# arrufat/zignal

Measured on NVIDIA H100. Metric: Mpixels/sec Gaussian-blur 8K RGBA f32, higher is better.
Workload: dtype f32

## Files before the change

zignal_b200/csrc/zb_conv_fused.cu:

```cuda
#include "zb_conv.h"
#include "zb_device.cuh"
#include "zb_shard.h"
#include "zb_tma.cuh"

namespace zb {

namespace {

constexpr int TW = 256;
constexpr int CHUNK = 8;
constexpr int G = TW / 8 + 2;
constexpr int STAGE_BYTES = G * CHUNK * 128;
constexpr int RING_ROWS = 24;
constexpr int RING_ROW_BYTES = TW * 16;
constexpr int RING_BYTES = RING_ROWS * RING_ROW_BYTES;
constexpr int NTHREADS = 256;
constexpr int MAX_HALF = 8;
constexpr int MAXK = 2 * MAX_HALF + 1;
constexpr int STAGES = 2;
constexpr int SMEM_BYTES = STAGES * STAGE_BYTES + RING_BYTES + 64 + 1024;

struct FusedParams {
    float kx[MAXK];
    float ky[MAXK];
    const float4* src;
    float4* dst;
    unsigned long long src_pitch_px, dst_pitch_px;
    int rows, cols, border;
    int ngroups;
    int n_strips;
    int n_units;
    int strip_lo, strip_hi;
    int n_segs, seg_chunks, seg_extra;
    int e_segs, e_chunks, e_extra;
    int row0, row1;
    int fix_rows;
    int fix_left;
    int fix_right;
    int tma_row_off;
    int edge_fast;
    int lsrc[8];
    int rsrc[8];
};

struct ShardParams {
    const float4* up_rows;
    const float4* down_rows;
    unsigned long long up_pitch_px, down_pitch_px;
    int half;
    ShardLink link;
};

template <bool ROTATE>
__device__ __forceinline__ void unit_at(const FusedParams& p, int u, int& strip, int& ra, int& rb) {
    const int n_inner = p.strip_hi - p.strip_lo;
    int seg, chunks, extra;
    if (u < p.n_segs * n_inner) {
        seg = u / n_inner;
        strip = p.strip_lo + (u - seg * n_inner);
        if constexpr (ROTATE) seg = seg + 1 == p.n_segs ? 0 : seg + 1;
        chunks = p.seg_chunks;
        extra = p.seg_extra;
    } else {
        const int n_edge = p.n_strips - n_inner;
        u -= p.n_segs * n_inner;
        seg = u / n_edge;
        const int e = u - seg * n_edge;
        strip = e < p.strip_lo ? e : e - p.strip_lo + p.strip_hi;
        chunks = p.e_chunks;
        extra = p.e_extra;
    }
    ra = p.row0 + (seg * chunks + min(seg, extra)) * CHUNK;
    rb = min(ra + (chunks + (seg < extra ? 1 : 0)) * CHUNK, p.row1);
}

template <bool EXACT>
__device__ __forceinline__ void mac4(float4& acc, const float4& v, float k) {
    if constexpr (EXACT) {
        acc.x = __fadd_rn(acc.x, __fmul_rn(v.x, k));
        acc.y = __fadd_rn(acc.y, __fmul_rn(v.y, k));
        acc.z = __fadd_rn(acc.z, __fmul_rn(v.z, k));
        acc.w = __fadd_rn(acc.w, __fmul_rn(v.w, k));
    } else {
        acc.x = fmaf(v.x, k, acc.x);
        acc.y = fmaf(v.y, k, acc.y);
        acc.z = fmaf(v.z, k, acc.z);
        acc.w = fmaf(v.w, k, acc.w);
    }
}

template <bool SHARD>
__device__ __noinline__ void fixup_stage(uint32_t stage, int y0, int xs0, bool fix_x, bool fix_rows, const FusedParams& p,
                                         int nb_lo, int nb_hi) {
    const int xlimit = p.ngroups * 8;
    auto stage_addr = [&](int rr, int xx) {
        const uint32_t line = (uint32_t)(rr * G + (xx >> 3));
        return stage + line * 128 + ((((uint32_t)xx & 7u) ^ (line & 7u)) << 4);
    };
    if (fix_x && p.edge_fast) {
        fix_x = false;
        if (threadIdx.x < 128) {
            const int side = threadIdx.x >> 6, rr = (threadIdx.x >> 3) & 7, e = threadIdx.x & 7;
            const int y = y0 + rr;
            bool row_ok = y >= 0 && y < p.rows;
            if constexpr (SHARD) row_ok = row_ok || (y < 0 && y >= nb_lo) || (y >= p.rows && y < nb_hi);
            const bool edge = side == 0 ? xs0 < 0 : xs0 + G * 8 > p.cols;
            if (row_ok && edge) {
                const int s_dst = side == 0 ? e : p.cols - xs0 + e;
                const int s_src = side == 0 ? p.lsrc[e] : p.rsrc[e] - xs0;
                if (s_dst < G * 8) sts128(stage_addr(rr, s_dst), lds128(stage_addr(rr, s_src)));
            }
        }
    }
    if (fix_x) {
        const int nleft = xs0 < 0 ? min(-xs0, G * 8) : 0;
        const int r0 = max(0, xlimit - xs0);
        const int r1 = min(G * 8, p.cols - xs0 + MAX_HALF);
        const int per_row = nleft + max(0, r1 - r0);
        for (int idx = threadIdx.x; idx < CHUNK * per_row; idx += NTHREADS) {
            const int rr = idx / per_row, e = idx - rr * per_row;
            const int xx = e < nleft ? e : r0 + (e - nleft);
            const int y = y0 + rr, x = xs0 + xx;
            const float4* rowp = p.src + (long long)y * (long long)p.src_pitch_px;
            if (y < 0 || y >= p.rows) {
                if constexpr (SHARD) {
                    if (y < nb_lo || y >= nb_hi) continue;
                } else {
                    continue;
                }
            }
            const int rx = resolve_index(x, p.cols, p.border);
            float4 v = make_float4(0.f, 0.f, 0.f, 0.f);
            if (rx >= 0) {
                const int sx = rx - xs0;
                if (rx < xlimit && sx >= 0 && sx < G * 8) v = lds128(stage_addr(rr, sx));
                else v = __ldg(rowp + rx);
            }
            sts128(stage_addr(rr, xx), v);
        }
    }
    if (fix_rows) {
        for (int idx = threadIdx.x; idx < CHUNK * G * 8; idx += NTHREADS) {
            const int rr = idx / (G * 8);
            const int xx = idx - rr * (G * 8);
            const int y = y0 + rr, x = xs0 + xx;
            if (y >= 0 && y < p.rows) continue;
            if constexpr (SHARD) {
                if (y >= nb_lo && y < nb_hi) continue;
            }
            const int ry = resolve_index(y, p.rows, p.border);
            const int rx = resolve_index(x, p.cols, p.border);
            float4 v = make_float4(0.f, 0.f, 0.f, 0.f);
            if (ry >= 0 && rx >= 0) v = __ldg(p.src + (size_t)ry * p.src_pitch_px + rx);
            sts128(stage_addr(rr, xx), v);
        }
    }
}

template <int HALF, bool EXACT, int SLOT>
__device__ __forceinline__ void v_pass(uint32_t v_col, const FusedParams& p, float4* out, bool col_ok, int rows_left) {
    constexpr int K = 2 * HALF + 1;
    constexpr int NLOAD = CHUNK + 2 * HALF;
    float4 acc[8];
#pragma unroll
    for (int o = 0; o < 8; ++o) acc[o] = make_float4(0.f, 0.f, 0.f, 0.f);
#pragma unroll
    for (int j = 0; j < NLOAD; ++j) {
        const int sr = (SLOT * CHUNK + 8 - HALF + j) % RING_ROWS;
        const float4 v = lds128(v_col + (uint32_t)(sr * RING_ROW_BYTES));
#pragma unroll
        for (int o = 0; o < 8; ++o) {
            const int ti = j - o;
            if (ti >= 0 && ti < K) mac4<EXACT>(acc[o], v, p.ky[ti]);
        }
    }
    if (col_ok) {
#pragma unroll
        for (int o = 0; o < 8; ++o)
            if (o < rows_left) __stcs(out + (size_t)o * p.dst_pitch_px, acc[o]);
    }
}

template <int HALF, bool EXACT, bool SHARD>
__device__ __forceinline__ uint32_t fused_units(const CUtensorMap& tmap, const FusedParams& p, unsigned nbr, int k_begin, int k_end, uint32_t count0) {
    constexpr int K = 2 * HALF + 1;
    constexpr int NLOAD = CHUNK + 2 * HALF;
    extern __shared__ unsigned char smem_raw[];
    const uint32_t smem0 = (smem_u32(smem_raw) + 1023u) & ~1023u;
    const uint32_t ring = smem0 + STAGES * STAGE_BYTES;
    const uint32_t bar0 = ring + RING_BYTES;

    const int tid = threadIdx.x;
    const long long u_first = (long long)blockIdx.x + (long long)k_begin * gridDim.x;
    const long long u_last = (long long)blockIdx.x + (long long)k_end * gridDim.x;
    const int n_units = (int)min((long long)p.n_units, u_last);
    if (u_first >= n_units) return count0;
    auto touches_neighbour = [&](int y) { return ((nbr & 1u) && y < 0) || ((nbr & 2u) && y + CHUNK > p.rows); };

    int pu = (int)u_first, pi = 0;
    uint32_t pcount = count0;
    auto produce = [&]() {
        if (pu >= n_units) return;
        int strip, ra, rb;
        unit_at<SHARD>(p, pu, strip, ra, rb);
        const int n_in = (rb - ra + CHUNK - 1) / CHUNK + 2;
        const uint32_t st = pcount % STAGES;
        const int y = ra - CHUNK + CHUNK * pi;
        fence_proxy_async();
        mbar_arrive_expect_tx(bar0 + 8 * st, STAGE_BYTES);
        tma_load_3d(smem0 + st * STAGE_BYTES, &tmap, 0, strip * (TW / 8) - 1, y + p.tma_row_off, bar0 + 8 * st);
        ++pcount;
        if (++pi == n_in) { pi = 0; pu += gridDim.x; }
    };
    if (tid == 0)
        for (int i = 0; i < STAGES; ++i) produce();

    const int ht = tid & 31, hr = tid >> 5;
    const int vx = tid;
    const uint32_t v_col = ring + (uint32_t)(vx >> 3) * 128u + ((((uint32_t)vx & 7u) ^ (((uint32_t)vx >> 3) & 7u)) << 4);
    const uint32_t h_ring_col = ring + (uint32_t)ht * 128u;
    const uint32_t h_key = (uint32_t)ht & 7u;

    uint32_t ccount = count0;

    for (int unit = (int)u_first; unit < n_units; unit += gridDim.x) {
        int strip, ra, rb;
        unit_at<SHARD>(p, unit, strip, ra, rb);
        const int x0 = strip * TW;
        const int n_out = (rb - ra + CHUNK - 1) / CHUNK;
        const int n_in = n_out + 2;
        const int g0 = x0 / 8 - 1;

        for (int i = 0; i < n_in; ++i, ++ccount) {
            const uint32_t st = ccount % STAGES;
            const uint32_t stage = smem0 + st * STAGE_BYTES;
            while (!mbar_try_wait(bar0 + 8 * st, (ccount / STAGES) & 1u)) {}
            const int y0 = ra - CHUNK + CHUNK * i;
            bool fix_r = p.fix_rows && (y0 < 0 || y0 + CHUNK > p.rows);
            if constexpr (SHARD) {
                if (touches_neighbour(y0)) fix_r = false;
            }
            const bool fix_x = (p.fix_left && g0 < 0) || (p.fix_right && (g0 + G) * 8 > p.ngroups * 8);
            if (fix_r || fix_x) {
                fixup_stage<SHARD>(stage, y0, g0 * 8, fix_x, fix_r, p, (nbr & 1u) ? INT_MIN : 0, (nbr & 2u) ? INT_MAX : p.rows);
                __syncthreads();
            }

            {
                const uint32_t line0 = (uint32_t)(hr * G + ht);
                uint32_t lbase[3];
#pragma unroll
                for (int l = 0; l < 3; ++l) lbase[l] = stage + (line0 + l) * 128u + (((line0 + l) & 7u) << 4);
                const uint32_t rrow = h_ring_col + (uint32_t)(((i % 3) * CHUNK + hr) * RING_ROW_BYTES);
                float4 acc[8];
#pragma unroll
                for (int o = 0; o < 8; ++o) acc[o] = make_float4(0.f, 0.f, 0.f, 0.f);
#pragma unroll
                for (int j = 0; j < NLOAD; ++j) {
                    const int pidx = 8 - HALF + j;
                    const float4 v = lds128(lbase[pidx >> 3] ^ (((uint32_t)pidx & 7u) << 4));
#pragma unroll
                    for (int o = 0; o < 8; ++o) {
                        const int ti = j - o;
                        if (ti >= 0 && ti < K) mac4<EXACT>(acc[o], v, p.kx[ti]);
                    }
                }
#pragma unroll
                for (int o = 0; o < 8; ++o) sts128(rrow + ((((uint32_t)o) ^ h_key) << 4), acc[o]);
            }
            __syncthreads();

            if (tid == 0) produce();

            if (i >= 2) {
                const int c = i - 2;
                const int x = x0 + vx;
                const int yb = ra + CHUNK * c;
                float4* out = p.dst + (size_t)yb * p.dst_pitch_px + x;
                const bool col_ok = x < p.cols;
                switch (c % 3) {
                    case 0: v_pass<HALF, EXACT, 0>(v_col, p, out, col_ok, rb - yb); break;
                    case 1: v_pass<HALF, EXACT, 1>(v_col, p, out, col_ok, rb - yb); break;
                    default: v_pass<HALF, EXACT, 2>(v_col, p, out, col_ok, rb - yb); break;
                }
            }
            __syncthreads();
        }
    }
    return ccount;
}

template <int HALF, bool EXACT, bool SHARD>
__device__ __forceinline__ void fused_sep_rgbaf32_body(const CUtensorMap& tmap, const FusedParams& p, const ShardParams* sp) {
    extern __shared__ unsigned char smem_raw[];
    const uint32_t smem0 = (smem_u32(smem_raw) + 1023u) & ~1023u;
    const uint32_t bar0 = smem0 + STAGES * STAGE_BYTES + RING_BYTES;
    const int tid = threadIdx.x;
    if (tid == 0) {
        asm volatile("prefetch.tensormap [%0];" ::"l"(&tmap) : "memory");
        for (int i = 0; i < STAGES; ++i) mbar_init(bar0 + 8 * i, 1);
        fence_barrier_init();
    }
    if constexpr (!SHARD) {
        __syncthreads();
        fused_units<HALF, EXACT, false>(tmap, p, 0u, 0, INT_MAX / 2048, 0u);
    } else {
        ShardCtrl* me = sp->link.self;
        const unsigned long long epoch = sp->link.epoch;
        const unsigned nbr = (sp->up_rows ? 1u : 0u) | (sp->down_rows ? 2u : 0u);
        const int per_side = sp->half * p.cols;
        const int total = (sp->up_rows ? per_side : 0) + (sp->down_rows ? per_side : 0);
        constexpr int BATCH = 12;
        const int rem = p.n_units % (int)gridDim.x;
        const int n_copiers = (int)gridDim.x - rem;
        const int ci = (int)blockIdx.x - rem;
        const bool copier = ci >= 0 && (long long)ci * NTHREADS * BATCH < total;
        if (tid == 0) {
            if (blockIdx.x == 0) {
                me->dbg[0] = global_timer_ns();
                if (sp->link.up) st_release_sys(&sp->link.up->ready_from[1], epoch);
                if (sp->link.down) st_release_sys(&sp->link.down->ready_from[0], epoch);
            }
            if (copier) {
                if (sp->up_rows) shard_wait_ge(&me->ready_from[0], epoch, me);
                if (sp->down_rows) shard_wait_ge(&me->ready_from[1], epoch, me);
                if (ci == 0) me->dbg[1] = global_timer_ns();
            }
        }
        __syncthreads();
        if (copier) {
            for (int base = ci * NTHREADS * BATCH; base < total; base += n_copiers * NTHREADS * BATCH) {
                float4 v[BATCH];
                float4* dstp[BATCH];
    #pragma unroll
                for (int k = 0; k < BATCH; ++k) {
                    int e = base + k * NTHREADS + tid;
                    dstp[k] = nullptr;
                    if (e < total) {
                        const bool upper = sp->up_rows && e < per_side;
                        if (!upper && sp->up_rows) e -= per_side;
                        const int r = e / p.cols, x = e - r * p.cols;
                        if (upper) {
                            v[k] = *(sp->up_rows + (size_t)r * sp->up_pitch_px + x);
                            dstp[k] = const_cast<float4*>(p.src) + (long long)(r - sp->half) * (long long)p.src_pitch_px + x;
                        } else {
                            v[k] = *(sp->down_rows + (size_t)r * sp->down_pitch_px + x);
                            dstp[k] = const_cast<float4*>(p.src) + (long long)(p.rows + r) * (long long)p.src_pitch_px + x;
                        }
                    }
                }
    #pragma unroll
                for (int k = 0; k < BATCH; ++k)
                    if (dstp[k]) *dstp[k] = v[k];
            }
            asm volatile("fence.proxy.async;" ::: "memory");
            __syncthreads();
        }
        if (tid == 0) {
            __threadfence();
            if (atomicAdd(&me->halo_reads[0], 1u) == gridDim.x - 1u) {
                me->halo_reads[0] = 0;
                me->dbg[2] = global_timer_ns();
                __threadfence();
                st_release_sys(&me->halo_landed, epoch);
                if (sp->up_rows) st_release_sys(&sp->link.up->done_from[1], epoch);
                if (sp->down_rows) st_release_sys(&sp->link.down->done_from[0], epoch);
            }
        }
        const long long first_halo_unit = (long long)max(0, p.n_segs - 2) * p.n_strips;
        const int k_split = first_halo_unit <= (long long)blockIdx.x ? 0 : (int)((first_halo_unit - blockIdx.x + gridDim.x - 1) / gridDim.x);
        const uint32_t count = fused_units<HALF, EXACT, true>(tmap, p, nbr, 0, k_split, 0u);
        if ((long long)blockIdx.x + (long long)k_split * gridDim.x < (long long)p.n_units) {
            if (tid == 0) {
                shard_wait_ge(&me->halo_landed, epoch, me);
                asm volatile("fence.proxy.async;" ::: "memory");
            }
            __syncthreads();
            fused_units<HALF, EXACT, true>(tmap, p, nbr, k_split, INT_MAX / 2048, count);
        }
        if (tid == 0) {
            ShardCtrl* me = sp->link.self;
            __threadfence();
            if (atomicAdd(&me->exit_ticket, 1u) == gridDim.x - 1u) {
                me->exit_ticket = 0;
                me->dbg[3] = global_timer_ns();
                if (sp->link.up) shard_wait_ge(&me->done_from[0], sp->link.epoch, me);
                if (sp->link.down) shard_wait_ge(&me->done_from[1], sp->link.epoch, me);
                me->dbg[4] = global_timer_ns();
            }
        }
    }
}


template <int HALF, bool EXACT>
__global__ void __launch_bounds__(NTHREADS, 1)
fused_sep_rgbaf32_kernel(const __grid_constant__ CUtensorMap tmap, const __grid_constant__ FusedParams p) {
    fused_sep_rgbaf32_body<HALF, EXACT, false>(tmap, p, nullptr);
}

template <int HALF, bool EXACT>
__global__ void __launch_bounds__(NTHREADS, 1)
fused_sep_rgbaf32_shard_kernel(const __grid_constant__ CUtensorMap tmap, const __grid_constant__ FusedParams p,
                               const __grid_constant__ ShardParams sp) {
    fused_sep_rgbaf32_body<HALF, EXACT, true>(tmap, p, &sp);
}

template <int HALF>
int launch_fused(const CUtensorMap& tmap, const FusedParams& p, const ShardParams* sp, int grid, bool exact, cudaStream_t s) {
    if (sp) {
        auto k = exact ? fused_sep_rgbaf32_shard_kernel<HALF, true> : fused_sep_rgbaf32_shard_kernel<HALF, false>;
        ZB_CUDA(cudaFuncSetAttribute(k, cudaFuncAttributeMaxDynamicSharedMemorySize, SMEM_BYTES));
        k<<<grid, NTHREADS, SMEM_BYTES, s>>>(tmap, p, *sp);
    } else {
        auto k = exact ? fused_sep_rgbaf32_kernel<HALF, true> : fused_sep_rgbaf32_kernel<HALF, false>;
        ZB_CUDA(cudaFuncSetAttribute(k, cudaFuncAttributeMaxDynamicSharedMemorySize, SMEM_BYTES));
        k<<<grid, NTHREADS, SMEM_BYTES, s>>>(tmap, p);
    }
    ZB_LAUNCHED();
    return ZB_OK;
}

int launch_half(int half, const CUtensorMap& tmap, const FusedParams& p, const ShardParams* sp, int grid, bool exact, cudaStream_t s) {
    switch (half) {
        case 1: return launch_fused<1>(tmap, p, sp, grid, exact, s);
        case 2: return launch_fused<2>(tmap, p, sp, grid, exact, s);
        case 3: return launch_fused<3>(tmap, p, sp, grid, exact, s);
        case 4: return launch_fused<4>(tmap, p, sp, grid, exact, s);
        case 5: return launch_fused<5>(tmap, p, sp, grid, exact, s);
        case 6: return launch_fused<6>(tmap, p, sp, grid, exact, s);
        case 7: return launch_fused<7>(tmap, p, sp, grid, exact, s);
        case 8: return launch_fused<8>(tmap, p, sp, grid, exact, s);
    }
    return ZB_ERR_UNSUPPORTED;
}

}

static int encode_block_map(EncodeTiledFn encode, CUtensorMap& tmap, void* data, int ngroups, int rows, uint64_t stride_px) {
    const cuuint64_t gdim[3] = {32, (cuuint64_t)ngroups, (cuuint64_t)rows};
    const cuuint64_t gstr[2] = {128, (cuuint64_t)stride_px * 16};
    const cuuint32_t box[3] = {32, (cuuint32_t)G, (cuuint32_t)CHUNK};
    const cuuint32_t estr[3] = {1, 1, 1};
    CUresult cr = encode(&tmap, CU_TENSOR_MAP_DATA_TYPE_FLOAT32, 3, data, gdim, gstr, box, estr, CU_TENSOR_MAP_INTERLEAVE_NONE,
                         CU_TENSOR_MAP_SWIZZLE_128B, CU_TENSOR_MAP_L2_PROMOTION_L2_256B, CU_TENSOR_MAP_FLOAT_OOB_FILL_NONE);
    if (cr != CUDA_SUCCESS) {
        snprintf(t_last_error, sizeof(t_last_error), "cuTensorMapEncodeTiled failed: %d", (int)cr);
        return ZB_ERR_UNSUPPORTED;
    }
    return ZB_OK;
}

constexpr long long EDGE_COST_NUM = 5, EDGE_COST_DEN = 4;

static void plan_units(int nrows, int sm_count, FusedParams& p) {
    const long long chunks = (nrows + CHUNK - 1) / CHUNK;
    const long long max_segs = chunks / 8 < 1 ? 1 : (chunks / 8 < sm_count ? chunks / 8 : sm_count);
    const long long n_inner = p.strip_hi - p.strip_lo, n_edge = p.n_strips - n_inner;
    auto steps = [&](long long segs) { return (chunks + segs - 1) / segs + 2; };
    long long best_cost = -1, best_units = 0, best_s = 1, best_e = 1;
    for (long long s = 1; s <= max_segs; ++s) {
        const long long waves = (s * p.n_strips + sm_count - 1) / sm_count;
        long long e = s;
        if (n_edge > 0) {
            long long e_max = (waves * sm_count - s * n_inner) / n_edge;
            if (e_max > max_segs) e_max = max_segs;
            while (e < e_max && EDGE_COST_NUM * steps(e) > EDGE_COST_DEN * steps(s)) ++e;
        }
        const long long inner = n_inner > 0 ? EDGE_COST_DEN * steps(s) : 0, edge = n_edge > 0 ? EDGE_COST_NUM * steps(e) : 0;
        const long long cost = waves * (inner > edge ? inner : edge), units = s * n_inner + e * n_edge;
        if (best_cost < 0 || cost < best_cost || (cost == best_cost && units < best_units)) {
            best_cost = cost;
            best_units = units;
            best_s = s;
            best_e = e;
        }
    }
    p.n_units = (int)best_units;
    p.n_segs = (int)best_s;
    p.seg_chunks = (int)(chunks / best_s);
    p.seg_extra = (int)(chunks % best_s);
    p.e_segs = (int)best_e;
    p.e_chunks = (int)(chunks / best_e);
    p.e_extra = (int)(chunks % best_e);
}

static int fused_prepare(const zb_image* src, zb_image* dst, const float* kx, int nx, const float* ky, int ny, int border, int row0, int row1,
                         bool bands, FusedParams& p, CUtensorMap& tmap, int& grid, int& half_out, EncodeTiledFn& encode) {
    const int half_x = nx / 2, half_y = ny / 2;
    const int half = half_x > half_y ? half_x : half_y;
    if (half < 1 || half > MAX_HALF) return ZB_ERR_UNSUPPORTED;
    if (src->cols < 16 || src->rows < 16) return ZB_ERR_UNSUPPORTED;
    if (images_overlap(src, dst, 16)) return ZB_ERR_UNSUPPORTED;
    if (((uintptr_t)src->data & 15u) || ((uintptr_t)dst->data & 15u)) return ZB_ERR_UNSUPPORTED;
    for (int i = 0; i < nx; ++i) if (fabsf(kx[i]) < 1e-10f) return ZB_ERR_UNSUPPORTED;
    for (int i = 0; i < ny; ++i) if (fabsf(ky[i]) < 1e-10f) return ZB_ERR_UNSUPPORTED;
    encode = encode_tiled_fn();
    if (!encode) return ZB_ERR_UNSUPPORTED;
    DeviceInfo di;
    int rc = device_info(&di);
    if (rc) return rc;
    if (di.smem_optin < (size_t)SMEM_BYTES) return ZB_ERR_UNSUPPORTED;

    memset(&p, 0, sizeof(p));
    for (int i = 0; i < nx; ++i) p.kx[i + (half - half_x)] = kx[i];
    for (int i = 0; i < ny; ++i) p.ky[i + (half - half_y)] = ky[i];
    p.src = (const float4*)src->data;
    p.dst = (float4*)dst->data;
    p.src_pitch_px = src->stride;
    p.dst_pitch_px = dst->stride;
    p.rows = (int)src->rows;
    p.cols = (int)src->cols;
    p.border = border;
    p.ngroups = p.cols / 8;
    p.n_strips = (p.cols + TW - 1) / TW;
    p.row0 = row0 < 0 ? 0 : row0;
    p.row1 = (row1 < 0 || row1 > p.rows) ? p.rows : row1;
    if (p.row1 <= p.row0) { grid = 0; return ZB_OK; }
    const int nrows = p.row1 - p.row0;
    p.fix_rows = border != ZB_BORDER_ZERO;
    p.fix_left = border != ZB_BORDER_ZERO;
    p.fix_right = (border != ZB_BORDER_ZERO) || (p.cols % 8 != 0);
    p.strip_lo = 0;
    p.strip_hi = p.n_strips;
    if (bands) {
        const BandPlan plan = plan_bands(nrows, p.n_strips, di.sm_count, g_tune_band_rows.load());
        p.n_segs = plan.n_bands;
        p.seg_chunks = plan.band_rows / CHUNK;
        p.n_units = p.n_segs * p.n_strips;
    } else {
        if (p.fix_left) p.strip_lo = 1;
        while (p.fix_right && p.strip_hi > p.strip_lo && (p.strip_hi - 1) * (TW / 8) - 1 + G > p.ngroups) --p.strip_hi;
        if (p.strip_hi <= p.strip_lo) { p.strip_lo = 0; p.strip_hi = p.n_strips; }
        plan_units(nrows, di.sm_count, p);
    }
    p.edge_fast = g_tune_edge_fast.load() && (border == ZB_BORDER_REPLICATE || border == ZB_BORDER_MIRROR) && p.cols % 8 == 0 && p.cols >= 16;
    for (int e = 0; e < 8; ++e) {
        const int xl = e - 8, xr = p.cols + e;
        p.lsrc[e] = 8 + (border == ZB_BORDER_REPLICATE ? 0 : -xl);
        p.rsrc[e] = border == ZB_BORDER_REPLICATE ? p.cols - 1 : 2 * (p.cols - 1) - xr;
    }

    if ((rc = encode_block_map(encode, tmap, src->data, p.ngroups, p.rows, src->stride))) return rc;
    grid = p.n_units < di.sm_count ? p.n_units : di.sm_count;
    half_out = half;
    return ZB_OK;
}

int conv_separable_fused_rgbaf32(const zb_image* src, zb_image* dst, const float* kx, int nx, const float* ky, int ny, int border,
                                 bool exact, cudaStream_t s, int row0, int row1) {
    FusedParams p;
    CUtensorMap tmap;
    EncodeTiledFn encode;
    int grid = 0, half = 0;
    int rc = fused_prepare(src, dst, kx, nx, ky, ny, border, row0, row1, false, p, tmap, grid, half, encode);
    if (rc || grid == 0) return rc;
    t_last_kernel = exact ? "fused_sep_rgbaf32_exact" : "fused_sep_rgbaf32";
    return launch_half(half, tmap, p, nullptr, grid, exact, s);
}

int conv_separable_fused_rgbaf32_shard(const zb_image* src, zb_image* dst, const float* kx, int nx, const float* ky, int ny, int border,
                                       bool exact, const PeerBlock& up, const PeerBlock& down, uint32_t halo_cap, const ShardLink& link,
                                       cudaStream_t s) {
    if (src->rows % CHUNK != 0 || halo_cap < (uint32_t)CHUNK) return ZB_ERR_UNSUPPORTED;
    FusedParams p;
    CUtensorMap tmap;
    EncodeTiledFn encode;
    int grid = 0, half = 0;
    int rc = fused_prepare(src, dst, kx, nx, ky, ny, border, 0, -1, true, p, tmap, grid, half, encode);
    if (rc) return rc;
    if (grid == 0) return ZB_ERR_UNSUPPORTED;
    const uint32_t hv = (uint32_t)(ny / 2);
    if ((up.data && (up.rows < hv || ((uintptr_t)up.data & 15u))) || (down.data && (down.rows < hv || ((uintptr_t)down.data & 15u))))
        return ZB_ERR_UNSUPPORTED;
    void* ext = (char*)src->data - (size_t)halo_cap * src->stride * 16;
    if ((rc = encode_block_map(encode, tmap, ext, p.ngroups, (int)(src->rows + 2 * halo_cap), src->stride))) return rc;
    p.tma_row_off = (int)halo_cap;
    p.fix_rows = 1;
    ShardParams sp;
    memset(&sp, 0, sizeof(sp));
    sp.half = (int)hv;
    if (up.data && hv) {
        sp.up_rows = (const float4*)up.data + (size_t)(up.rows - hv) * up.stride;
        sp.up_pitch_px = up.stride;
    }
    if (down.data && hv) {
        sp.down_rows = (const float4*)down.data;
        sp.down_pitch_px = down.stride;
    }
    sp.link = link;
    if (!sp.up_rows) sp.link.up = nullptr;
    if (!sp.down_rows) sp.link.down = nullptr;
    {
        DeviceInfo di;
        if ((rc = device_info(&di))) return rc;
        grid = di.sm_count;
    }
    t_last_kernel = exact ? "fused_sep_rgbaf32_shard_exact" : "fused_sep_rgbaf32_shard";
    return launch_half(half, tmap, p, &sp, grid, exact, s);
}

}
```

zignal_b200/csrc/zb_internal.h:

```cpp
#pragma once
#include <cuda.h>
#include <cuda_runtime.h>

#include <atomic>
#include <cstdint>
#include <cstdio>
#include <cstring>

#include "../../include/zignal_b200.h"

namespace zb {

extern std::atomic<uint64_t> g_launches;
extern thread_local char t_last_error[512];
extern thread_local const char* t_last_kernel;
extern std::atomic<int> g_exact_f32;
extern std::atomic<int> g_force_generic;
extern std::atomic<int> g_tune_band_rows;
extern std::atomic<int> g_tune_host_band_rows;
extern std::atomic<int> g_tune_edge_fast;
extern std::atomic<int> g_tune_sobel_tile;
extern std::atomic<int> g_tune_jacobi_cluster;
extern std::atomic<int> g_tune_u8_dp;
extern std::atomic<int> g_tune_u8_fmath;
extern std::atomic<int> g_tune_hough_threads;
extern std::atomic<int> g_tune_hough_max_cols;
extern std::atomic<int> g_tune_dither_publish;

int set_cuda_error(cudaError_t e, const char* what, const char* file, int line);

#define ZB_CUDA(expr)                                                                    \
    do {                                                                                 \
        cudaError_t _e = (expr);                                                         \
        if (_e != cudaSuccess) return ::zb::set_cuda_error(_e, #expr, __FILE__, __LINE__); \
    } while (0)

#define ZB_LAUNCHED()                                                                      \
    do {                                                                                   \
        ::zb::g_launches.fetch_add(1, std::memory_order_relaxed);                          \
        cudaError_t _e = cudaGetLastError();                                               \
        if (_e != cudaSuccess) return ::zb::set_cuda_error(_e, "kernel launch", __FILE__, __LINE__); \
    } while (0)

struct DeviceInfo {
    int ordinal = -1;
    int sm_count = 0;
    size_t smem_optin = 0;
};
int device_info(DeviceInfo* out);
typedef CUresult (*EncodeTiledFn)(CUtensorMap*, CUtensorMapDataType, cuuint32_t, void*, const cuuint64_t*, const cuuint64_t*,
                                  const cuuint32_t*, const cuuint32_t*, CUtensorMapInterleave, CUtensorMapSwizzle,
                                  CUtensorMapL2promotion, CUtensorMapFloatOOBfill);
EncodeTiledFn encode_tiled_fn();

static inline int channels_of(int pixfmt) {
    switch (pixfmt) {
        case ZB_PIX_U8: case ZB_PIX_F32: return 1;
        case ZB_PIX_RGB8: return 3;
        case ZB_PIX_RGBA8: case ZB_PIX_RGBAF32: return 4;
    }
    return 0;
}
static inline size_t channel_bytes(int pixfmt) { return (pixfmt == ZB_PIX_F32 || pixfmt == ZB_PIX_RGBAF32) ? 4 : 1; }
static inline size_t pixel_bytes(int pixfmt) { return (size_t)channels_of(pixfmt) * channel_bytes(pixfmt); }
static inline bool is_float_fmt(int pixfmt) { return pixfmt == ZB_PIX_F32 || pixfmt == ZB_PIX_RGBAF32; }

struct Scratch {
    void* p = nullptr;
    cudaStream_t s = nullptr;
    ~Scratch() { if (p) cudaFreeAsync(p, s); }
    int alloc(size_t bytes, cudaStream_t stream);
    template <typename T> T* as() const { return (T*)p; }
// ... 34 lines not shown
```

zignal_b200/csrc/zb_runtime.cu:

```cuda
#include <mutex>

#include "zb_internal.h"

namespace zb {

std::atomic<uint64_t> g_launches{0};
thread_local char t_last_error[512] = "";
thread_local const char* t_last_kernel = "";
std::atomic<int> g_exact_f32{0};
std::atomic<int> g_force_generic{0};
std::atomic<int> g_tune_band_rows{256};
std::atomic<int> g_tune_host_band_rows{256};
std::atomic<int> g_tune_u8_fmath{1};
std::atomic<int> g_tune_u8_dp{1};
std::atomic<int> g_tune_rotate_tile{1};
std::atomic<int> g_tune_edge_fast{1};
std::atomic<int> g_tune_sobel_tile{1};
std::atomic<int> g_tune_jacobi_cluster{1};

int set_cuda_error(cudaError_t e, const char* what, const char* file, int line) {
    snprintf(t_last_error, sizeof(t_last_error), "%s: %s (%s:%d)", cudaGetErrorName(e), what, file, line);
    if (e == cudaErrorMemoryAllocation) return ZB_ERR_OUT_OF_MEMORY;
    return ZB_ERR_DEVICE_FAILURE;
}

static std::mutex g_mu;
static DeviceInfo g_dev[64];
static EncodeTiledFn g_encode = nullptr;

int device_info(DeviceInfo* out) {
    int dev = 0;
    ZB_CUDA(cudaGetDevice(&dev));
    if (dev < 0 || dev >= 64) return ZB_ERR_DEVICE_FAILURE;
    std::lock_guard<std::mutex> lk(g_mu);
    if (g_dev[dev].ordinal != dev) {
        cudaDeviceProp prop;
        ZB_CUDA(cudaGetDeviceProperties(&prop, dev));
        g_dev[dev].sm_count = prop.multiProcessorCount;
        g_dev[dev].smem_optin = prop.sharedMemPerBlockOptin;
        cudaMemPool_t pool;
        ZB_CUDA(cudaDeviceGetDefaultMemPool(&pool, dev));
        uint64_t thresh = UINT64_MAX;
        ZB_CUDA(cudaMemPoolSetAttribute(pool, cudaMemPoolAttrReleaseThreshold, &thresh));
        g_dev[dev].ordinal = dev;
    }
    *out = g_dev[dev];
    return ZB_OK;
}

EncodeTiledFn encode_tiled_fn() {
    std::lock_guard<std::mutex> lk(g_mu);
    if (!g_encode) {
        void* fn = nullptr;
        cudaDriverEntryPointQueryResult qres;
        if (cudaGetDriverEntryPoint("cuTensorMapEncodeTiled", &fn, cudaEnableDefault, &qres) == cudaSuccess &&
            qres == cudaDriverEntryPointSuccess)
            g_encode = (EncodeTiledFn)fn;
    }
    return g_encode;
}

int Scratch::alloc(size_t bytes, cudaStream_t stream) {
    s = stream;
    if (bytes == 0) bytes = 16;
    ZB_CUDA(cudaMallocAsync(&p, bytes, stream));
    return ZB_OK;
}

}

using namespace zb;

extern "C" {

int zb_version(void) { return ZB_VERSION_MAJOR * 1000 + ZB_VERSION_MINOR; }

const char* zb_status_name(int status) {
    switch (status) {
        case ZB_OK: return "Ok";
        case ZB_ERR_DIMENSION_MISMATCH: return "DimensionMismatch";
        case ZB_ERR_INVALID_SIGMA: return "InvalidSigma";
        case ZB_ERR_UNSUPPORTED: return "Unsupported";
        case ZB_ERR_NOT_CONVERGED: return "NotConverged";
        case ZB_ERR_INVALID_ARGUMENT: return "InvalidArgument";
        case ZB_ERR_OUT_OF_MEMORY: return "OutOfMemory";
        case ZB_ERR_DEVICE_FAILURE: return "DeviceFailure";
        case ZB_ERR_INVALID_SCALE_FACTOR: return "InvalidScaleFactor";
        case ZB_ERR_INVALID_DIMENSIONS: return "InvalidDimensions";
        case ZB_ERR_NO_TARGET_SET: return "NoTargetSet";
        case ZB_ERR_NO_SOURCE_SET: return "NoSourceSet";
        case ZB_ERR_INSUFFICIENT_DATA: return "InsufficientData";
        case ZB_ERR_INVALID_COMPONENTS: return "InvalidComponents";
        case ZB_ERR_INVALID_THRESHOLD: return "InvalidThreshold";
        case ZB_ERR_INVALID_PERCENTILE: return "InvalidPercentile";
        case ZB_ERR_INVALID_TRIM: return "InvalidTrim";
        case ZB_ERR_IMAGE_TOO_SMALL: return "ImageTooSmall";
        case ZB_ERR_NOT_SQUARE: return "NotSquare";
        case ZB_ERR_NOT_SYMMETRIC: return "NotSymmetric";
        case ZB_ERR_NOT_FINITE: return "NotFinite";
        case ZB_ERR_INVALID_CUTOFF: return "InvalidCutoff";
        case ZB_ERR_INVALID_RADIUS: return "InvalidRadius";
        case ZB_ERR_INVALID_KERNEL_SIZE: return "InvalidKernelSize";
        case ZB_ERR_INVALID_B_PARAMETER: return "InvalidBParameter";
        case ZB_ERR_WINDOW_SIZE_MUST_BE_ODD: return "WindowSizeMustBeOdd";
        case ZB_ERR_WINDOW_SIZE_TOO_SMALL: return "WindowSizeTooSmall";
        case ZB_ERR_OUT_OF_BOUNDS: return "OutOfBounds";
        case ZB_ERR_NO_PALETTE_COLORS: return "NoPaletteColors";
    }
    return "Unknown";
}

const char* zb_last_error(void) { return t_last_error; }
const char* zb_last_kernel(void) { return t_last_kernel; }
uint64_t zb_kernel_launch_count(void) { return g_launches.load(); }
int zb_set_exact_f32(int on) { g_exact_f32.store(on ? 1 : 0); return ZB_OK; }
int zb_set_force_generic(int on) { g_force_generic.store(on ? 1 : 0); return ZB_OK; }
int zb_tune(const char* key, int value) {
    if (!key) return ZB_ERR_INVALID_ARGUMENT;
    if (!strcmp(key, "conv.u8_fmath")) { g_tune_u8_fmath.store(value ? 1 : 0); return ZB_OK; }
    if (!strcmp(key, "conv.u8_dp")) { g_tune_u8_dp.store(value ? 1 : 0); return ZB_OK; }
    if (!strcmp(key, "conv.edge_fast")) { g_tune_edge_fast.store(value ? 1 : 0); return ZB_OK; }
    if (!strcmp(key, "sobel.tile")) { g_tune_sobel_tile.store(value ? 1 : 0); return ZB_OK; }
    if (!strcmp(key, "jacobi.cluster")) { g_tune_jacobi_cluster.store(value ? 1 : 0); return ZB_OK; }
    if (!strcmp(key, "rotate.tile")) { g_tune_rotate_tile.store(value ? 1 : 0); return ZB_OK; }
    if (!strcmp(key, "host.band_rows")) { if (value < 0) return ZB_ERR_INVALID_ARGUMENT; g_tune_host_band_rows.store(value); return ZB_OK; }
    if (!strcmp(key, "conv.band_rows")) { if (value < 64) return ZB_ERR_INVALID_ARGUMENT; g_tune_band_rows.store(value); return ZB_OK; }
    if (!strcmp(key, "hough.threads")) {
        if (value < 128 || value > 1024 || value % 32) return ZB_ERR_INVALID_ARGUMENT;
        g_tune_hough_threads.store(value);
        return ZB_OK;
    }
    if (!strcmp(key, "hough.max_cols")) { if (value < 1) return ZB_ERR_INVALID_ARGUMENT; g_tune_hough_max_cols.store(value); return ZB_OK; }
    if (!strcmp(key, "dither.publish")) {
        if (value < 1 || value > 4096) return ZB_ERR_INVALID_ARGUMENT;
        g_tune_dither_publish.store(value);
        return ZB_OK;
    }
    return ZB_ERR_INVALID_ARGUMENT;
}

int zb_device_count(int* count) { ZB_CUDA(cudaGetDeviceCount(count)); return ZB_OK; }
int zb_set_device(int ordinal) { ZB_CUDA(cudaSetDevice(ordinal)); return ZB_OK; }
int zb_get_device(int* ordinal) { ZB_CUDA(cudaGetDevice(ordinal)); return ZB_OK; }
int zb_sm_count(int* count) {
    DeviceInfo di;
    int rc = device_info(&di);
    if (rc) return rc;
    *count = di.sm_count;
    return ZB_OK;
}

int zb_stream_create(zb_stream* out) {
    cudaStream_t s;
    ZB_CUDA(cudaStreamCreateWithFlags(&s, cudaStreamNonBlocking));
    *out = (zb_stream)s;
    return ZB_OK;
}
int zb_stream_destroy(zb_stream s) { ZB_CUDA(cudaStreamDestroy((cudaStream_t)s)); return ZB_OK; }
int zb_stream_synchronize(zb_stream s) { ZB_CUDA(cudaStreamSynchronize((cudaStream_t)s)); return ZB_OK; }

int zb_malloc(void** out, size_t bytes, zb_stream s) {
    DeviceInfo di;
    int rc = device_info(&di);
    if (rc) return rc;
    if (bytes == 0) bytes = 16;
    ZB_CUDA(cudaMallocAsync(out, bytes, (cudaStream_t)s));
    return ZB_OK;
}
int zb_free(void* p, zb_stream s) {
    if (!p) return ZB_OK;
    ZB_CUDA(cudaFreeAsync(p, (cudaStream_t)s));
    return ZB_OK;
}
int zb_malloc_host(void** out, size_t bytes) {
// ... 52 lines not shown
```

Measured before the change: 85580.

## Add 128-pixel strip variant of fused RGBA f32 blur with multi-CTA occupancy

Templates the fused separable blur kernel on strip width so a 128-pixel strip and 128-thread CTA variant can run several CTAs per SM. The grid and unit planner scale with CTAs-per-SM slots and use a different edge cost ratio for narrow strips. The default strip width stays 256, so the new path runs only when the tune key selects it. The change also turns off TMA L2 promotion for the non-shard path, which does affect the default run.

```diff
diff --git a/zignal_b200/csrc/zb_conv_fused.cu b/zignal_b200/csrc/zb_conv_fused.cu
--- a/zignal_b200/csrc/zb_conv_fused.cu
+++ b/zignal_b200/csrc/zb_conv_fused.cu
@@ -7,18 +7,22 @@
 
 namespace {
 
-constexpr int TW = 256;
 constexpr int CHUNK = 8;
-constexpr int G = TW / 8 + 2;
-constexpr int STAGE_BYTES = G * CHUNK * 128;
 constexpr int RING_ROWS = 24;
-constexpr int RING_ROW_BYTES = TW * 16;
-constexpr int RING_BYTES = RING_ROWS * RING_ROW_BYTES;
-constexpr int NTHREADS = 256;
 constexpr int MAX_HALF = 8;
 constexpr int MAXK = 2 * MAX_HALF + 1;
 constexpr int STAGES = 2;
-constexpr int SMEM_BYTES = STAGES * STAGE_BYTES + RING_BYTES + 64 + 1024;
+
+template <int TW>
+struct Strip {
+    static constexpr int NTHREADS = TW;
+    static constexpr int G = TW / 8 + 2;
+    static constexpr int STAGE_BYTES = G * CHUNK * 128;
+    static constexpr int RING_ROW_BYTES = TW * 16;
+    static constexpr int RING_BYTES = RING_ROWS * RING_ROW_BYTES;
+    static constexpr int SMEM_BYTES = STAGES * STAGE_BYTES + RING_BYTES + 64 + 1024;
+};
+static_assert(Strip<128>::STAGE_BYTES % 1024 == 0 && Strip<256>::STAGE_BYTES % 1024 == 0, "stages must stay 1 KB aligned");
 
 struct FusedParams {
     float kx[MAXK];
@@ -89,9 +93,10 @@
     }
 }
 
-template <bool SHARD>
+template <int TW, bool SHARD>
 __device__ __noinline__ void fixup_stage(uint32_t stage, int y0, int xs0, bool fix_x, bool fix_rows, const FusedParams& p,
                                          int nb_lo, int nb_hi) {
+    constexpr int G = Strip<TW>::G, NTHREADS = Strip<TW>::NTHREADS;
     const int xlimit = p.ngroups * 8;
     auto stage_addr = [&](int rr, int xx) {
         const uint32_t line = (uint32_t)(rr * G + (xx >> 3));
@@ -157,7 +162,7 @@
     }
 }
 
-template <int HALF, bool EXACT, int SLOT>
+template <int TW, int HALF, bool EXACT, int SLOT>
 __device__ __forceinline__ void v_pass(uint32_t v_col, const FusedParams& p, float4* out, bool col_ok, int rows_left) {
     constexpr int K = 2 * HALF + 1;
     constexpr int NLOAD = CHUNK + 2 * HALF;
@@ -167,7 +172,7 @@
 #pragma unroll
     for (int j = 0; j < NLOAD; ++j) {
         const int sr = (SLOT * CHUNK + 8 - HALF + j) % RING_ROWS;
-        const float4 v = lds128(v_col + (uint32_t)(sr * RING_ROW_BYTES));
+        const float4 v = lds128(v_col + (uint32_t)(sr * Strip<TW>::RING_ROW_BYTES));
 #pragma unroll
         for (int o = 0; o < 8; ++o) {
             const int ti = j - o;
@@ -181,14 +186,16 @@
     }
 }
 
-template <int HALF, bool EXACT, bool SHARD>
+template <int TW, int HALF, bool EXACT, bool SHARD>
 __device__ __forceinline__ uint32_t fused_units(const CUtensorMap& tmap, const FusedParams& p, unsigned nbr, int k_begin, int k_end, uint32_t count0) {
+    using L = Strip<TW>;
+    constexpr int G = L::G, STAGE_BYTES = L::STAGE_BYTES, RING_ROW_BYTES = L::RING_ROW_BYTES;
     constexpr int K = 2 * HALF + 1;
     constexpr int NLOAD = CHUNK + 2 * HALF;
     extern __shared__ unsigned char smem_raw[];
     const uint32_t smem0 = (smem_u32(smem_raw) + 1023u) & ~1023u;
     const uint32_t ring = smem0 + STAGES * STAGE_BYTES;
-    const uint32_t bar0 = ring + RING_BYTES;
+    const uint32_t bar0 = ring + L::RING_BYTES;
 
     const int tid = threadIdx.x;
     const long long u_first = (long long)blockIdx.x + (long long)k_begin * gridDim.x;
@@ -215,7 +222,9 @@
     if (tid == 0)
         for (int i = 0; i < STAGES; ++i) produce();
 
-    const int ht = tid & 31, hr = tid >> 5;
+    constexpr int ROW_SHIFT = TW == 256 ? 5 : 4;
+    static_assert(TW / 8 == 1 << ROW_SHIFT, "strips of 128 or 256 pixels");
+    const int ht = tid & (TW / 8 - 1), hr = tid >> ROW_SHIFT;
     const int vx = tid;
     const uint32_t v_col = ring + (uint32_t)(vx >> 3) * 128u + ((((uint32_t)vx & 7u) ^ (((uint32_t)vx >> 3) & 7u)) << 4);
     const uint32_t h_ring_col = ring + (uint32_t)ht * 128u;
@@ -242,7 +251,7 @@
             }
             const bool fix_x = (p.fix_left && g0 < 0) || (p.fix_right && (g0 + G) * 8 > p.ngroups * 8);
             if (fix_r || fix_x) {
-                fixup_stage<SHARD>(stage, y0, g0 * 8, fix_x, fix_r, p, (nbr & 1u) ? INT_MIN : 0, (nbr & 2u) ? INT_MAX : p.rows);
+                fixup_stage<TW, SHARD>(stage, y0, g0 * 8, fix_x, fix_r, p, (nbr & 1u) ? INT_MIN : 0, (nbr & 2u) ? INT_MAX : p.rows);
                 __syncthreads();
             }
 
@@ -279,9 +288,9 @@
                 float4* out = p.dst + (size_t)yb * p.dst_pitch_px + x;
                 const bool col_ok = x < p.cols;
                 switch (c % 3) {
-                    case 0: v_pass<HALF, EXACT, 0>(v_col, p, out, col_ok, rb - yb); break;
-                    case 1: v_pass<HALF, EXACT, 1>(v_col, p, out, col_ok, rb - yb); break;
-                    default: v_pass<HALF, EXACT, 2>(v_col, p, out, col_ok, rb - yb); break;
+                    case 0: v_pass<TW, HALF, EXACT, 0>(v_col, p, out, col_ok, rb - yb); break;
+                    case 1: v_pass<TW, HALF, EXACT, 1>(v_col, p, out, col_ok, rb - yb); break;
+                    default: v_pass<TW, HALF, EXACT, 2>(v_col, p, out, col_ok, rb - yb); break;
                 }
             }
             __syncthreads();
@@ -290,11 +299,12 @@
     return ccount;
 }
 
-template <int HALF, bool EXACT, bool SHARD>
+template <int TW, int HALF, bool EXACT, bool SHARD>
 __device__ __forceinline__ void fused_sep_rgbaf32_body(const CUtensorMap& tmap, const FusedParams& p, const ShardParams* sp) {
+    constexpr int NTHREADS = Strip<TW>::NTHREADS;
     extern __shared__ unsigned char smem_raw[];
     const uint32_t smem0 = (smem_u32(smem_raw) + 1023u) & ~1023u;
-    const uint32_t bar0 = smem0 + STAGES * STAGE_BYTES + RING_BYTES;
+    const uint32_t bar0 = smem0 + STAGES * Strip<TW>::STAGE_BYTES + Strip<TW>::RING_BYTES;
     const int tid = threadIdx.x;
     if (tid == 0) {
         asm volatile("prefetch.tensormap [%0];" ::"l"(&tmap) : "memory");
@@ -303,7 +313,7 @@
     }
     if constexpr (!SHARD) {
         __syncthreads();
-        fused_units<HALF, EXACT, false>(tmap, p, 0u, 0, INT_MAX / 2048, 0u);
+        fused_units<TW, HALF, EXACT, false>(tmap, p, 0u, 0, INT_MAX / 2048, 0u);
     } else {
         ShardCtrl* me = sp->link.self;
         const unsigned long long epoch = sp->link.epoch;
@@ -369,14 +379,14 @@
         }
         const long long first_halo_unit = (long long)max(0, p.n_segs - 2) * p.n_strips;
         const int k_split = first_halo_unit <= (long long)blockIdx.x ? 0 : (int)((first_halo_unit - blockIdx.x + gridDim.x - 1) / gridDim.x);
-        const uint32_t count = fused_units<HALF, EXACT, true>(tmap, p, nbr, 0, k_split, 0u);
+        const uint32_t count = fused_units<TW, HALF, EXACT, true>(tmap, p, nbr, 0, k_split, 0u);
         if ((long long)blockIdx.x + (long long)k_split * gridDim.x < (long long)p.n_units) {
             if (tid == 0) {
                 shard_wait_ge(&me->halo_landed, epoch, me);
                 asm volatile("fence.proxy.async;" ::: "memory");
             }
             __syncthreads();
-            fused_units<HALF, EXACT, true>(tmap, p, nbr, k_split, INT_MAX / 2048, count);
+            fused_units<TW, HALF, EXACT, true>(tmap, p, nbr, k_split, INT_MAX / 2048, count);
         }
         if (tid == 0) {
             ShardCtrl* me = sp->link.self;
@@ -393,57 +403,91 @@
 }
 
 
+template <int TW, int HALF, bool EXACT>
+__global__ void __launch_bounds__(Strip<TW>::NTHREADS, 256 / TW)
+fused_sep_rgbaf32_kernel(const __grid_constant__ CUtensorMap tmap, const __grid_constant__ FusedParams p) {
+    fused_sep_rgbaf32_body<TW, HALF, EXACT, false>(tmap, p, nullptr);
+}
+
 template <int HALF, bool EXACT>
-__global__ void __launch_bounds__(NTHREADS, 1)
-fused_sep_rgbaf32_kernel(const __grid_constant__ CUtensorMap tmap, const __grid_constant__ FusedParams p) {
-    fused_sep_rgbaf32_body<HALF, EXACT, false>(tmap, p, nullptr);
-}
-
-template <int HALF, bool EXACT>
-__global__ void __launch_bounds__(NTHREADS, 1)
+__global__ void __launch_bounds__(Strip<256>::NTHREADS, 1)
 fused_sep_rgbaf32_shard_kernel(const __grid_constant__ CUtensorMap tmap, const __grid_constant__ FusedParams p,
                                const __grid_constant__ ShardParams sp) {
-    fused_sep_rgbaf32_body<HALF, EXACT, true>(tmap, p, &sp);
-}
-
-template <int HALF>
-int launch_fused(const CUtensorMap& tmap, const FusedParams& p, const ShardParams* sp, int grid, bool exact, cudaStream_t s) {
-    if (sp) {
-        auto k = exact ? fused_sep_rgbaf32_shard_kernel<HALF, true> : fused_sep_rgbaf32_shard_kernel<HALF, false>;
-        ZB_CUDA(cudaFuncSetAttribute(k, cudaFuncAttributeMaxDynamicSharedMemorySize, SMEM_BYTES));
-        k<<<grid, NTHREADS, SMEM_BYTES, s>>>(tmap, p, *sp);
-    } else {
-        auto k = exact ? fused_sep_rgbaf32_kernel<HALF, true> : fused_sep_rgbaf32_kernel<HALF, false>;
-        ZB_CUDA(cudaFuncSetAttribute(k, cudaFuncAttributeMaxDynamicSharedMemorySize, SMEM_BYTES));
-        k<<<grid, NTHREADS, SMEM_BYTES, s>>>(tmap, p);
-    }
+    fused_sep_rgbaf32_body<256, HALF, EXACT, true>(tmap, p, &sp);
+}
+
+template <int TW, int HALF, bool EXACT>
+int launch_single(const CUtensorMap& tmap, const FusedParams& p, int grid, cudaStream_t s) {
+    using L = Strip<TW>;
+    auto k = fused_sep_rgbaf32_kernel<TW, HALF, EXACT>;
+    ZB_CUDA(cudaFuncSetAttribute(k, cudaFuncAttributeMaxDynamicSharedMemorySize, L::SMEM_BYTES));
+    k<<<grid, L::NTHREADS, L::SMEM_BYTES, s>>>(tmap, p);
     ZB_LAUNCHED();
     return ZB_OK;
 }
 
-int launch_half(int half, const CUtensorMap& tmap, const FusedParams& p, const ShardParams* sp, int grid, bool exact, cudaStream_t s) {
+template <int HALF>
+int launch_fused(int tw, const CUtensorMap& tmap, const FusedParams& p, const ShardParams* sp, int grid, bool exact, cudaStream_t s) {
+    if (sp) {
+        using L = Strip<256>;
+        auto k = exact ? fused_sep_rgbaf32_shard_kernel<HALF, true> : fused_sep_rgbaf32_shard_kernel<HALF, false>;
+        ZB_CUDA(cudaFuncSetAttribute(k, cudaFuncAttributeMaxDynamicSharedMemorySize, L::SMEM_BYTES));
+        k<<<grid, L::NTHREADS, L::SMEM_BYTES, s>>>(tmap, p, *sp);
+        ZB_LAUNCHED();
+        return ZB_OK;
+    }
+    if (tw == 128) return exact ? launch_single<128, HALF, true>(tmap, p, grid, s) : launch_single<128, HALF, false>(tmap, p, grid, s);
+    return exact ? launch_single<256, HALF, true>(tmap, p, grid, s) : launch_single<256, HALF, false>(tmap, p, grid, s);
+}
+
+int launch_half(int half, int tw, const CUtensorMap& tmap, const FusedParams& p, const ShardParams* sp, int grid, bool exact, cudaStream_t s) {
     switch (half) {
-        case 1: return launch_fused<1>(tmap, p, sp, grid, exact, s);
-        case 2: return launch_fused<2>(tmap, p, sp, grid, exact, s);
-        case 3: return launch_fused<3>(tmap, p, sp, grid, exact, s);
-        case 4: return launch_fused<4>(tmap, p, sp, grid, exact, s);
-        case 5: return launch_fused<5>(tmap, p, sp, grid, exact, s);
-        case 6: return launch_fused<6>(tmap, p, sp, grid, exact, s);
-        case 7: return launch_fused<7>(tmap, p, sp, grid, exact, s);
-        case 8: return launch_fused<8>(tmap, p, sp, grid, exact, s);
+        case 1: return launch_fused<1>(tw, tmap, p, sp, grid, exact, s);
+        case 2: return launch_fused<2>(tw, tmap, p, sp, grid, exact, s);
+        case 3: return launch_fused<3>(tw, tmap, p, sp, grid, exact, s);
+        case 4: return launch_fused<4>(tw, tmap, p, sp, grid, exact, s);
+        case 5: return launch_fused<5>(tw, tmap, p, sp, grid, exact, s);
+        case 6: return launch_fused<6>(tw, tmap, p, sp, grid, exact, s);
+        case 7: return launch_fused<7>(tw, tmap, p, sp, grid, exact, s);
+        case 8: return launch_fused<8>(tw, tmap, p, sp, grid, exact, s);
     }
     return ZB_ERR_UNSUPPORTED;
 }
 
-}
-
-static int encode_block_map(EncodeTiledFn encode, CUtensorMap& tmap, void* data, int ngroups, int rows, uint64_t stride_px) {
+template <int HALF>
+int ctas_per_sm_128(bool exact, int* n) {
+    using L = Strip<128>;
+    auto k = exact ? fused_sep_rgbaf32_kernel<128, HALF, true> : fused_sep_rgbaf32_kernel<128, HALF, false>;
+    ZB_CUDA(cudaFuncSetAttribute(k, cudaFuncAttributeMaxDynamicSharedMemorySize, L::SMEM_BYTES));
+    ZB_CUDA(cudaOccupancyMaxActiveBlocksPerMultiprocessor(n, k, L::NTHREADS, L::SMEM_BYTES));
+    return ZB_OK;
+}
+
+int ctas_per_sm_half(int half, bool exact, int* n) {
+    switch (half) {
+        case 1: return ctas_per_sm_128<1>(exact, n);
+        case 2: return ctas_per_sm_128<2>(exact, n);
+        case 3: return ctas_per_sm_128<3>(exact, n);
+        case 4: return ctas_per_sm_128<4>(exact, n);
+        case 5: return ctas_per_sm_128<5>(exact, n);
+        case 6: return ctas_per_sm_128<6>(exact, n);
+        case 7: return ctas_per_sm_128<7>(exact, n);
+        case 8: return ctas_per_sm_128<8>(exact, n);
+    }
+    return ZB_ERR_UNSUPPORTED;
+}
+
+}
+
+template <int TW>
+static int encode_block_map(EncodeTiledFn encode, CUtensorMap& tmap, void* data, int ngroups, int rows, uint64_t stride_px,
+                            CUtensorMapL2promotion promotion) {
     const cuuint64_t gdim[3] = {32, (cuuint64_t)ngroups, (cuuint64_t)rows};
     const cuuint64_t gstr[2] = {128, (cuuint64_t)stride_px * 16};
-    const cuuint32_t box[3] = {32, (cuuint32_t)G, (cuuint32_t)CHUNK};
+    const cuuint32_t box[3] = {32, (cuuint32_t)Strip<TW>::G, (cuuint32_t)CHUNK};
     const cuuint32_t estr[3] = {1, 1, 1};
     CUresult cr = encode(&tmap, CU_TENSOR_MAP_DATA_TYPE_FLOAT32, 3, data, gdim, gstr, box, estr, CU_TENSOR_MAP_INTERLEAVE_NONE,
-                         CU_TENSOR_MAP_SWIZZLE_128B, CU_TENSOR_MAP_L2_PROMOTION_L2_256B, CU_TENSOR_MAP_FLOAT_OOB_FILL_NONE);
+                         CU_TENSOR_MAP_SWIZZLE_128B, promotion, CU_TENSOR_MAP_FLOAT_OOB_FILL_NONE);
     if (cr != CUDA_SUCCESS) {
         snprintf(t_last_error, sizeof(t_last_error), "cuTensorMapEncodeTiled failed: %d", (int)cr);
         return ZB_ERR_UNSUPPORTED;
@@ -452,8 +496,10 @@
 }
 
 constexpr long long EDGE_COST_NUM = 5, EDGE_COST_DEN = 4;
-
-static void plan_units(int nrows, int sm_count, FusedParams& p) {
+constexpr long long EDGE_COST_NUM_128 = 7, EDGE_COST_DEN_128 = 4;
+
+static void plan_units(int nrows, int sm_count, int tw, FusedParams& p) {
+    const long long edge_num = tw == 128 ? EDGE_COST_NUM_128 : EDGE_COST_NUM, edge_den = tw == 128 ? EDGE_COST_DEN_128 : EDGE_COST_DEN;
     const long long chunks = (nrows + CHUNK - 1) / CHUNK;
     const long long max_segs = chunks / 8 < 1 ? 1 : (chunks / 8 < sm_count ? chunks / 8 : sm_count);
     const long long n_inner = p.strip_hi - p.strip_lo, n_edge = p.n_strips - n_inner;
@@ -465,9 +511,9 @@
         if (n_edge > 0) {
             long long e_max = (waves * sm_count - s * n_inner) / n_edge;
             if (e_max > max_segs) e_max = max_segs;
-            while (e < e_max && EDGE_COST_NUM * steps(e) > EDGE_COST_DEN * steps(s)) ++e;
-        }
-        const long long inner = n_inner > 0 ? EDGE_COST_DEN * steps(s) : 0, edge = n_edge > 0 ? EDGE_COST_NUM * steps(e) : 0;
+            while (e < e_max && edge_num * steps(e) > edge_den * steps(s)) ++e;
+        }
+        const long long inner = n_inner > 0 ? edge_den * steps(s) : 0, edge = n_edge > 0 ? edge_num * steps(e) : 0;
         const long long cost = waves * (inner > edge ? inner : edge), units = s * n_inner + e * n_edge;
         if (best_cost < 0 || cost < best_cost || (cost == best_cost && units < best_units)) {
             best_cost = cost;
@@ -486,7 +532,8 @@
 }
 
 static int fused_prepare(const zb_image* src, zb_image* dst, const float* kx, int nx, const float* ky, int ny, int border, int row0, int row1,
-                         bool bands, FusedParams& p, CUtensorMap& tmap, int& grid, int& half_out, EncodeTiledFn& encode) {
+                         bool bands, int tw, int ctas_per_sm, FusedParams& p, CUtensorMap& tmap, int& grid, int& half_out,
+                         EncodeTiledFn& encode) {
     const int half_x = nx / 2, half_y = ny / 2;
     const int half = half_x > half_y ? half_x : half_y;
     if (half < 1 || half > MAX_HALF) return ZB_ERR_UNSUPPORTED;
@@ -500,7 +547,8 @@
     DeviceInfo di;
     int rc = device_info(&di);
     if (rc) return rc;
-    if (di.smem_optin < (size_t)SMEM_BYTES) return ZB_ERR_UNSUPPORTED;
+    if (di.smem_optin < (size_t)(tw == 128 ? Strip<128>::SMEM_BYTES : Strip<256>::SMEM_BYTES)) return ZB_ERR_UNSUPPORTED;
+    const int slots = ctas_per_sm * di.sm_count;
 
     memset(&p, 0, sizeof(p));
     for (int i = 0; i < nx; ++i) p.kx[i + (half - half_x)] = kx[i];
@@ -513,7 +561,7 @@
     p.cols = (int)src->cols;
     p.border = border;
     p.ngroups = p.cols / 8;
-    p.n_strips = (p.cols + TW - 1) / TW;
+    p.n_strips = (p.cols + tw - 1) / tw;
     p.row0 = row0 < 0 ? 0 : row0;
     p.row1 = (row1 < 0 || row1 > p.rows) ? p.rows : row1;
     if (p.row1 <= p.row0) { grid = 0; return ZB_OK; }
@@ -530,9 +578,9 @@
         p.n_units = p.n_segs * p.n_strips;
     } else {
         if (p.fix_left) p.strip_lo = 1;
-        while (p.fix_right && p.strip_hi > p.strip_lo && (p.strip_hi - 1) * (TW / 8) - 1 + G > p.ngroups) --p.strip_hi;
+        while (p.fix_right && p.strip_hi > p.strip_lo && (p.strip_hi - 1) * (tw / 8) - 1 + (tw / 8 + 2) > p.ngroups) --p.strip_hi;
         if (p.strip_hi <= p.strip_lo) { p.strip_lo = 0; p.strip_hi = p.n_strips; }
-        plan_units(nrows, di.sm_count, p);
+        plan_units(nrows, slots, tw, p);
     }
     p.edge_fast = g_tune_edge_fast.load() && (border == ZB_BORDER_REPLICATE || border == ZB_BORDER_MIRROR) && p.cols % 8 == 0 && p.cols >= 16;
     for (int e = 0; e < 8; ++e) {
@@ -541,22 +589,30 @@
         p.rsrc[e] = border == ZB_BORDER_REPLICATE ? p.cols - 1 : 2 * (p.cols - 1) - xr;
     }
 
-    if ((rc = encode_block_map(encode, tmap, src->data, p.ngroups, p.rows, src->stride))) return rc;
-    grid = p.n_units < di.sm_count ? p.n_units : di.sm_count;
+    rc = tw == 128 ? encode_block_map<128>(encode, tmap, src->data, p.ngroups, p.rows, src->stride, CU_TENSOR_MAP_L2_PROMOTION_NONE)
+                   : encode_block_map<256>(encode, tmap, src->data, p.ngroups, p.rows, src->stride, CU_TENSOR_MAP_L2_PROMOTION_NONE);
+    if (rc) return rc;
+    grid = p.n_units < slots ? p.n_units : slots;
     half_out = half;
     return ZB_OK;
 }
 
 int conv_separable_fused_rgbaf32(const zb_image* src, zb_image* dst, const float* kx, int nx, const float* ky, int ny, int border,
                                  bool exact, cudaStream_t s, int row0, int row1) {
+    int tw = g_tune_strip_px.load(), ctas_per_sm = 1, rc;
+    if (tw == 128) {
+        const int half = nx / 2 > ny / 2 ? nx / 2 : ny / 2;
+        if ((rc = ctas_per_sm_half(half, exact, &ctas_per_sm))) return rc;
+        if (ctas_per_sm < 2) { tw = 256; ctas_per_sm = 1; }
+    }
     FusedParams p;
     CUtensorMap tmap;
     EncodeTiledFn encode;
     int grid = 0, half = 0;
-    int rc = fused_prepare(src, dst, kx, nx, ky, ny, border, row0, row1, false, p, tmap, grid, half, encode);
+    rc = fused_prepare(src, dst, kx, nx, ky, ny, border, row0, row1, false, tw, ctas_per_sm, p, tmap, grid, half, encode);
     if (rc || grid == 0) return rc;
     t_last_kernel = exact ? "fused_sep_rgbaf32_exact" : "fused_sep_rgbaf32";
-    return launch_half(half, tmap, p, nullptr, grid, exact, s);
+    return launch_half(half, tw, tmap, p, nullptr, grid, exact, s);
 }
 
 int conv_separable_fused_rgbaf32_shard(const zb_image* src, zb_image* dst, const float* kx, int nx, const float* ky, int ny, int border,
@@ -567,14 +623,15 @@
     CUtensorMap tmap;
     EncodeTiledFn encode;
     int grid = 0, half = 0;
-    int rc = fused_prepare(src, dst, kx, nx, ky, ny, border, 0, -1, true, p, tmap, grid, half, encode);
+    int rc = fused_prepare(src, dst, kx, nx, ky, ny, border, 0, -1, true, 256, 1, p, tmap, grid, half, encode);
     if (rc) return rc;
     if (grid == 0) return ZB_ERR_UNSUPPORTED;
     const uint32_t hv = (uint32_t)(ny / 2);
     if ((up.data && (up.rows < hv || ((uintptr_t)up.data & 15u))) || (down.data && (down.rows < hv || ((uintptr_t)down.data & 15u))))
         return ZB_ERR_UNSUPPORTED;
     void* ext = (char*)src->data - (size_t)halo_cap * src->stride * 16;
-    if ((rc = encode_block_map(encode, tmap, ext, p.ngroups, (int)(src->rows + 2 * halo_cap), src->stride))) return rc;
+    if ((rc = encode_block_map<256>(encode, tmap, ext, p.ngroups, (int)(src->rows + 2 * halo_cap), src->stride, CU_TENSOR_MAP_L2_PROMOTION_L2_256B)))
+        return rc;
     p.tma_row_off = (int)halo_cap;
     p.fix_rows = 1;
     ShardParams sp;
@@ -597,7 +654,7 @@
         grid = di.sm_count;
     }
     t_last_kernel = exact ? "fused_sep_rgbaf32_shard_exact" : "fused_sep_rgbaf32_shard";
-    return launch_half(half, tmap, p, &sp, grid, exact, s);
-}
-
-}
+    return launch_half(half, 256, tmap, p, &sp, grid, exact, s);
+}
+
+}
diff --git a/zignal_b200/csrc/zb_internal.h b/zignal_b200/csrc/zb_internal.h
--- a/zignal_b200/csrc/zb_internal.h
+++ b/zignal_b200/csrc/zb_internal.h
@@ -18,6 +18,7 @@
 extern std::atomic<int> g_force_generic;
 extern std::atomic<int> g_tune_band_rows;
 extern std::atomic<int> g_tune_host_band_rows;
+extern std::atomic<int> g_tune_strip_px;
 extern std::atomic<int> g_tune_edge_fast;
 extern std::atomic<int> g_tune_sobel_tile;
 extern std::atomic<int> g_tune_jacobi_cluster;
diff --git a/zignal_b200/csrc/zb_runtime.cu b/zignal_b200/csrc/zb_runtime.cu
--- a/zignal_b200/csrc/zb_runtime.cu
+++ b/zignal_b200/csrc/zb_runtime.cu
@@ -15,6 +15,7 @@
 std::atomic<int> g_tune_u8_dp{1};
 std::atomic<int> g_tune_rotate_tile{1};
 std::atomic<int> g_tune_edge_fast{1};
+std::atomic<int> g_tune_strip_px{256};
 std::atomic<int> g_tune_sobel_tile{1};
 std::atomic<int> g_tune_jacobi_cluster{1};
 
@@ -120,6 +121,7 @@
     if (!strcmp(key, "conv.u8_fmath")) { g_tune_u8_fmath.store(value ? 1 : 0); return ZB_OK; }
     if (!strcmp(key, "conv.u8_dp")) { g_tune_u8_dp.store(value ? 1 : 0); return ZB_OK; }
     if (!strcmp(key, "conv.edge_fast")) { g_tune_edge_fast.store(value ? 1 : 0); return ZB_OK; }
+    if (!strcmp(key, "conv.strip_px")) { if (value != 128 && value != 256) return ZB_ERR_INVALID_ARGUMENT; g_tune_strip_px.store(value); return ZB_OK; }
     if (!strcmp(key, "sobel.tile")) { g_tune_sobel_tile.store(value ? 1 : 0); return ZB_OK; }
     if (!strcmp(key, "jacobi.cluster")) { g_tune_jacobi_cluster.store(value ? 1 : 0); return ZB_OK; }
     if (!strcmp(key, "rotate.tile")) { g_tune_rotate_tile.store(value ? 1 : 0); return ZB_OK; }
```

Result: no change. 85240 (median of 6 runs) (-0.4%).
